# Linyou/Ced-NeRF

Measured on NVIDIA B200. Metric: train_step_rays_per_s, higher is better.
Workload: dtype f16 (MLP, tables) / f32 (marching, compositing, grads)

## Files before the change

### cednerf_b200/csrc/field_common.cuh

```cuda
#pragma once
#include "hashgrid.cuh"
#include "tc05.cuh"

struct CednerfFieldDesc {
  float aabb[6];
  float moving_step;
  int use_div_offsets;
  int time_mode;
  int time_before_sigma;
  CednerfMlpDesc f1, f2, f3;
  CednerfMlpDesc f4;
  CednerfGridLevels levels;
};

namespace {

__device__ __forceinline__ void group_sync(int group) { asm volatile("bar.sync %0, 128;" ::"r"(group + 1) : "memory"); }

__device__ __forceinline__ void run_chain(const CednerfMlpDesc& d, const uint8_t* wimg, uint8_t* abuf, uint32_t tmem_grp,
                                          uint32_t tmem_warp, uint64_t* bar, uint32_t& phase, int gtid, int group,
                                          uint8_t* save = nullptr, int64_t save_layer_stride = 0, int64_t save_row0 = 0,
                                          int save_rows = 0, uint8_t* save_in = nullptr) {

  const int L = d.n_layers;
  for (int l = 0; l < L; ++l) {
    const int K = d.dim_in[l], N = d.dim_out[l];
    if (gtid == 0) {
      tc_fence_after();
      const uint64_t ad = make_desc(smem_u32(abuf), 1, 64);
      const uint64_t bd = make_desc(smem_u32(wimg + d.image_off[l]), 1, 64);
      const uint32_t id = make_idesc(128, N, 0, 0);
      for (int k = 0; k < K / 16; ++k) umma(tmem_grp, ad + 2 * k, bd + 2 * k, id, k > 0);
      umma_commit(bar);
    }
    if (save_in && l == 0) {
      const int cpr = K >> 3;
      uint4* dst = reinterpret_cast<uint4*>(save_in + save_row0 * K * 2);
      for (int q = gtid; q < MLP_TILE * cpr; q += MLP_TILE) {
        const int r = q / cpr, c = q - r * cpr;
        if (r < save_rows) dst[q] = *reinterpret_cast<const uint4*>(abuf + swz(r, c));
      }
    }
    if (save && l > 0 && gtid == 0) {
      uint8_t* dst = save + ((int64_t)(l - 1) * save_layer_stride + (save_row0 >> 7)) * MLP_TILE_BYTES;
      asm volatile("cp.async.bulk.global.shared::cta.bulk_group [%0], [%1], %2;" ::"l"(dst), "r"(smem_u32(abuf)),
                   "r"((uint32_t)MLP_TILE_BYTES)
                   : "memory");
      asm volatile("cp.async.bulk.commit_group;" ::: "memory");
    }
    if ((gtid >> 5) == 0) {
      mbar_wait(bar, phase);
      tc_fence_after();
      tc_fence_before();
      if (save && l > 0 && gtid == 0) asm volatile("cp.async.bulk.wait_group.read 0;" ::: "memory");
    }
    group_sync(group);
    phase ^= 1;
    tc_fence_after();
    if (l < L - 1) {
#pragma unroll
      for (int cb = 0; cb < 4; ++cb) {
        uint32_t r[16];
        tmem_ld16(tmem_warp + cb * 16, r);
        tmem_ld_wait();
        uint32_t p[8];
#pragma unroll
        for (int j = 0; j < 8; ++j) p[j] = pack_relu_h2(__uint_as_float(r[2 * j]), __uint_as_float(r[2 * j + 1]));
        *reinterpret_cast<uint4*>(abuf + swz(gtid, 2 * cb)) = make_uint4(p[0], p[1], p[2], p[3]);
        *reinterpret_cast<uint4*>(abuf + swz(gtid, 2 * cb + 1)) = make_uint4(p[4], p[5], p[6], p[7]);
      }
      fence_proxy_async();
      tc_fence_before();
      group_sync(group);
    }
  }
}

__device__ __forceinline__ float rnd16(uint32_t acc_bits) { return __half2float(__float2half_rn(__uint_as_float(acc_bits))); }

template <bool EXACT = false>
__device__ __forceinline__ void time_embedding(float tv, float mvnorm, int mode, float* e ) {
  const float half_pi = 1.5707963267948966f;
  e[0] = tv;
  if (mode == 1) {
#pragma unroll
    for (int i = 0; i < 4; ++i) {
      const float tb = tv * (float)(1 << i);
      e[1 + i] = EXACT ? sinf(tb) : __sinf(tb);
      e[5 + i] = EXACT ? sinf(tb + half_pi) : __sinf(tb + half_pi);
    }
  } else {
    const float scm[4] = {0.f, 2.f, 8.f, 24.f};
#pragma unroll
    for (int i = 0; i < 4; ++i) {
      const float tb = tv * (float)(1 << i);
      const float att = EXACT ? expf(-1.f * (mvnorm * scm[i])) : __expf(-1.f * (mvnorm * scm[i]));
      e[1 + 2 * i] = (EXACT ? sinf(tb) : __sinf(tb)) * att;
      e[2 + 2 * i] = (EXACT ? sinf(tb + half_pi) : __sinf(tb + half_pi)) * att;
    }
  }
}

__device__ __noinline__ uint32_t wrapped_corner(uint32_t base, int k, uint32_t res, uint32_t r2, uint32_t size) {
  const uint32_t h = base + (uint32_t)(k & 1) + (uint32_t)((k >> 1) & 1) * res + (uint32_t)(k >> 2) * r2;
  return h >= size ? h % size : h;
}

__device__ __forceinline__ __half2 ldg_last(const __half2* p) {
  uint32_t v;
  asm("ld.global.nc.L1::evict_last.b32 %0, [%1];" : "=r"(v) : "l"(p));
  return *reinterpret_cast<__half2*>(&v);
}
__device__ __forceinline__ __half2 gather_h2(const __half2* base, uint32_t idx) {
  uint64_t addr;
  asm("mad.wide.u32 %0, %1, 4, %2;" : "=l"(addr) : "r"(idx), "l"(base));
  uint32_t v;
  asm("ld.global.nc.L1::evict_last.b32 %0, [%1];" : "=r"(v) : "l"(addr));
  return *reinterpret_cast<__half2*>(&v);
}

__device__ __forceinline__ uint64_t pack_f2(float a, float b) {
  uint64_t r;
  asm("mov.b64 %0, {%1, %2};" : "=l"(r) : "f"(a), "f"(b));
  return r;
}
__device__ __forceinline__ void unpack_f2(uint64_t v, float& a, float& b) { asm("mov.b64 {%0, %1}, %2;" : "=f"(a), "=f"(b) : "l"(v)); }
__device__ __forceinline__ uint64_t sub_f2(uint64_t a, uint64_t b) {
  uint64_t r;
  asm("sub.f32x2 %0, %1, %2;" : "=l"(r) : "l"(a), "l"(b));
  return r;
}
__device__ __forceinline__ uint64_t fma_f2(uint64_t a, uint64_t b, uint64_t c) {
  uint64_t r;
  asm("fma.rn.f32x2 %0, %1, %2, %3;" : "=l"(r) : "l"(a), "l"(b), "l"(c));
  return r;
}
__device__ __forceinline__ uint64_t h2_to_f2(__half2 h) {
  const float2 f = __half22float2(h);
  return pack_f2(f.x, f.y);
}

#ifndef HASH_PAIR_LOADS
#define HASH_PAIR_LOADS 1
#endif
#ifndef HASH_PAIR_MIN_RES
#define HASH_PAIR_MIN_RES 1024u
#endif
template <int LG>
__device__ __forceinline__ void hash_issue(const float* xn, const __half* __restrict__ table, const CednerfGridLevels& lv,
                                           int l_first, float (*frac)[3], __half2 (*v)[8]) {
#pragma unroll
  for (int a = 0; a < LG; ++a) {
// ... 154 lines not shown
```

### cednerf_b200/csrc/field_train.cu

```cuda
#include <stdlib.h>

#include "field_common.cuh"

namespace {

struct SavedLayout {
  int64_t h1, o1, in2, h2, o2, h3, h4, o4, xn, total, tiles;
};

__host__ __device__ inline SavedLayout saved_layout(const CednerfFieldDesc& d, int64_t n) {
  SavedLayout s;
  int64_t off = 0;
  const int64_t tiles = (n + MLP_TILE - 1) / MLP_TILE;
  s.tiles = tiles;
  s.h1 = off, off += (int64_t)(d.f1.n_layers - 1) * tiles * MLP_TILE_BYTES;
  s.o1 = off, off += n * 32;
  s.in2 = off, off += n * d.f2.dim_in[0] * 2;
  s.h2 = off, off += (int64_t)(d.f2.n_layers - 1) * tiles * MLP_TILE_BYTES;
  s.o2 = off, off += n * 32;
  s.h3 = off, off += (int64_t)(d.f3.n_layers - 1) * tiles * MLP_TILE_BYTES;
  s.h4 = off, off += d.f4.n_layers > 0 ? (int64_t)(d.f4.n_layers - 1) * tiles * MLP_TILE_BYTES : 0;
  s.o4 = off, off += d.f4.n_layers > 0 ? n * 64 : 0;
  s.xn = off, off += (n * 12 + 15) / 16 * 16;
  s.total = off;
  return s;
}

struct BwdWorkLayout {
  int64_t d_o2, d_in2, d_in4, g_xn, dy_lm, total;
};

__host__ __device__ inline BwdWorkLayout bwd_layout(const CednerfFieldDesc& d, int64_t n) {
  BwdWorkLayout w;
  int64_t off = 0;
  w.d_o2 = off, off += n * 32;
  w.d_in2 = off, off += n * d.f2.dim_in[0] * 2;
  w.d_in4 = off, off += n * 64;
  w.g_xn = off, off += (n * 12 + 15) / 16 * 16;
  w.dy_lm = off, off += (int64_t)d.levels.n_levels * n * 4;
  w.total = off;
  return w;
}

struct TrainArgs {
  const int64_t* ridx;
  const float* t0;
  const float* t1;
  const float* rays_o;
  const float* rays_d;
  const float* t;
  int t_stride;
  int64_t n;
  const int64_t* n_dev;
  const uint8_t* img[4];
  const __half* table;
  float* sigma;
  float* rgb;
  float* latent;
  uint8_t* selector;
  float* move;
  uint8_t* saved;
  const float* d_sigma;
  const float* d_rgb;
  const float* d_latent;
  uint8_t* work;
  float* d_params[4];
  uint32_t tmem_cols;
  int flush_tiles;
  const int32_t* order;
  CednerfFieldDesc d;
};

__device__ __forceinline__ int64_t ext_index(const TrainArgs& a, int64_t s) { return a.order ? (int64_t)a.order[s] : s; }

__device__ __forceinline__ int64_t live_count(const TrainArgs& a) {
  if (!a.n_dev) return a.n;
  const int64_t v = *a.n_dev;
  return v < a.n ? v : a.n;
}

__device__ __forceinline__ float huber(float x) {
  const float ax = fabsf(x);
  return ax < 1.f ? 0.5f * x * x : ax - 0.5f;
}

__device__ __forceinline__ void load_off(const TrainArgs& a, const SavedLayout& sl, int64_t s, float* off6) {
  const uint4 w = *reinterpret_cast<const uint4*>(a.saved + sl.o1 + s * 32);
  const uint32_t ww[4] = {w.x, w.y, w.z, w.w};
#pragma unroll
  for (int j = 0; j < 3; ++j) {
    const float2 f = __half22float2(*reinterpret_cast<const __half2*>(&ww[j]));
    off6[2 * j] = f.x;
    off6[2 * j + 1] = f.y;
  }
}

#ifdef FIELD_PHASE_CLOCKS
__device__ unsigned long long g_train_phase_clocks[12];
#define TPHASE_MARK(i)                                                           \
  do {                                                                           \
    if (gtid == 0) {                                                             \
      const long long now_ = clock64();                                          \
      atomicAdd(&g_train_phase_clocks[i], (unsigned long long)(now_ - phase_t)); \
      phase_t = now_;                                                            \
    }                                                                            \
  } while (0)
#else
#define TPHASE_MARK(i) do {} while (0)
#endif

#ifndef TRAIN_FWD_GROUPS
#define TRAIN_FWD_GROUPS 5
#endif
#ifndef TRAIN_FWD_LG
#define TRAIN_FWD_LG 4
#endif
__global__ void __launch_bounds__(TRAIN_FWD_GROUPS * 128, 1) field_train_fwd_kernel(TrainArgs a) {
  extern __shared__ __align__(1024) uint8_t smem_raw[];
  uint8_t* smem = reinterpret_cast<uint8_t*>((reinterpret_cast<uintptr_t>(smem_raw) + 1023) & ~(uintptr_t)1023);
  const CednerfFieldDesc& d = a.d;
  const bool has4 = d.f4.n_layers > 0;
  const int n_groups = blockDim.x / MLP_TILE;
  const int tid = threadIdx.x, warp = tid >> 5, group = tid / MLP_TILE, gtid = tid % MLP_TILE;
  uint8_t* w1 = smem;
  uint8_t* w2 = w1 + d.f1.image_bytes;
  uint8_t* w3 = w2 + d.f2.image_bytes;
  uint8_t* w4 = w3 + d.f3.image_bytes;
  uint8_t* abuf = reinterpret_cast<uint8_t*>(
                      (reinterpret_cast<uintptr_t>(w4 + (has4 ? d.f4.image_bytes : 0)) + 1023) & ~(uintptr_t)1023) +
                  (size_t)group * MLP_TILE_BYTES;
  __shared__ uint64_t bars[8];
  __shared__ uint32_t tmem_base_s;
  uint64_t* bar = &bars[group];
  {
    const uint8_t* src[4] = {a.img[0], a.img[1], a.img[2], a.img[3]};
    uint8_t* dst[4] = {w1, w2, w3, w4};
    const int bytes[4] = {d.f1.image_bytes, d.f2.image_bytes, d.f3.image_bytes, has4 ? d.f4.image_bytes : 0};
    for (int k = 0; k < 4; ++k)
      for (int q = tid; q < bytes[k] / 16; q += blockDim.x)
        reinterpret_cast<uint4*>(dst[k])[q] = __ldg(reinterpret_cast<const uint4*>(src[k]) + q);
  }
  const uint32_t tmem_cols = n_groups <= 1 ? 64 : (n_groups == 2 ? 128 : (n_groups <= 4 ? 256 : 512));
  if (warp == 0) tmem_alloc(&tmem_base_s, tmem_cols);
  if (gtid == 0) mbar_init(bar, 1);
  if (tid == 0) fence_barrier_init();
  fence_proxy_async();
  tc_fence_before();
  __syncthreads();
  tc_fence_after();
  const uint32_t tmem_base = tmem_base_s + 64u * (uint32_t)group;
  const uint32_t tmem_warp = tmem_base + ((uint32_t)((warp & 3) * 32) << 16);
  uint32_t phase = 0;
  const int64_t n = a.n, nl = live_count(a);
  const int64_t n_tiles = (nl + MLP_TILE - 1) / MLP_TILE;
  const int L = d.levels.n_levels;
  const uint32_t one2 = 0x3C003C00u;
  const SavedLayout sl = saved_layout(d, n);
  const int k2 = d.f2.dim_in[0];

  for (int64_t tile = blockIdx.x + (int64_t)gridDim.x * group; tile < n_tiles; tile += (int64_t)gridDim.x * n_groups) {
    const int64_t s = tile * MLP_TILE + gtid;
    const bool ok = s < nl;
    const int rows_valid = (int)((nl - tile * MLP_TILE) < MLP_TILE ? (nl - tile * MLP_TILE) : MLP_TILE);
    float x[3] = {0.f, 0.f, 0.f}, tv = 0.f;
    int64_t ray = 0;
#ifdef FIELD_PHASE_CLOCKS
    long long phase_t = clock64();
    if (gtid == 0) atomicAdd(&g_train_phase_clocks[11], 1ull);
#endif
    const int64_t e = ok ? ext_index(a, s) : 0;
    if (ok) packed_sample(a.ridx, a.t0, a.t1, a.rays_o, a.rays_d, a.t, a.t_stride, e, x, tv, ray);
    frequency_row<true>(abuf, gtid, x[0], x[1], x[2], tv);
    fence_proxy_async();
    tc_fence_before();
    group_sync(group);
    TPHASE_MARK(0);
    run_chain(d.f1, w1, abuf, tmem_base, tmem_warp, bar, phase, gtid, group, a.saved + sl.h1,
              sl.tiles, tile * MLP_TILE, rows_valid);
    TPHASE_MARK(1);
    float xn[3], mv[3], mvnorm;
    bool selector;
    {
      uint32_t r[16];
      tmem_ld16(tmem_warp, r);
      tmem_ld_wait();
      uint32_t p[8];
#pragma unroll
      for (int j = 0; j < 8; ++j) p[j] = pack_h2(__uint_as_float(r[2 * j]), __uint_as_float(r[2 * j + 1]));
      if (ok) {
        uint4* dst = reinterpret_cast<uint4*>(a.saved + sl.o1 + s * 32);
        dst[0] = make_uint4(p[0], p[1], p[2], p[3]);
        dst[1] = make_uint4(p[4], p[5], p[6], p[7]);
      }
      float off6[6];
#pragma unroll
      for (int k = 0; k < 6; ++k) off6[k] = rnd16(r[k]);
      apply_move(d, x, off6, mv, xn, selector);
      mvnorm = sqrtf(mv[0] * mv[0] + mv[1] * mv[1] + mv[2] * mv[2]);
    }
    if (ok) {
      float* xs = reinterpret_cast<float*>(a.saved + sl.xn) + 3 * s;
      xs[0] = xn[0], xs[1] = xn[1], xs[2] = xn[2];
      a.move[3 * e] = mv[0], a.move[3 * e + 1] = mv[1], a.move[3 * e + 2] = mv[2];
      a.selector[e] = (uint8_t)selector;
    }
    TPHASE_MARK(2);
    float temb[9];
    {
      auto put_word = [&](int w, uint32_t v) {
        *reinterpret_cast<uint32_t*>(abuf + swz(gtid, w >> 2) + ((w & 3) << 2)) = v;
      };
      if ((L % TRAIN_FWD_LG) == 0 && (L & 3) == 0) {
#pragma unroll 1
        for (int l0 = 0; l0 < L; l0 += TRAIN_FWD_LG) {
          uint32_t fw[TRAIN_FWD_LG];
          hash_levels<TRAIN_FWD_LG>(xn, a.table, d.levels, 0, fw, l0);
          if constexpr (TRAIN_FWD_LG >= 4) {
#pragma unroll
            for (int q = 0; q < TRAIN_FWD_LG / 4; ++q)
              *reinterpret_cast<uint4*>(abuf + swz(gtid, (l0 >> 2) + q)) = make_uint4(fw[4 * q], fw[4 * q + 1], fw[4 * q + 2], fw[4 * q + 3]);
          } else {
            *reinterpret_cast<uint2*>(abuf + swz(gtid, l0 >> 2) + ((l0 & 2) << 2)) = make_uint2(fw[0], fw[1]);
          }
        }
      } else {
#pragma unroll 1
        for (int l0 = 0; l0 < L; ++l0) {
          uint32_t f1w[1];
          hash_levels<1>(xn, a.table, d.levels, 0, f1w, l0);
          put_word(l0, f1w[0]);
        }
      }
      TPHASE_MARK(3);
      if (d.time_mode) time_embedding<true>(tv, mvnorm, d.time_mode, temb);
      int w = L;
      if (d.time_mode && d.time_before_sigma) {
#pragma unroll
        for (int j = 0; j < 4; ++j) put_word(L + j, pack_h2(temb[2 * j], temb[2 * j + 1]));
        put_word(L + 4, pack_h2(temb[8], 1.f));
        w = L + 5;
      }
      for (; 2 * w < k2; ++w) put_word(w, one2);
    }
    fence_proxy_async();
    tc_fence_before();
    group_sync(group);
    TPHASE_MARK(4);
    run_chain(d.f2, w2, abuf, tmem_base, tmem_warp, bar, phase, gtid, group, a.saved + sl.h2,
              sl.tiles, tile * MLP_TILE, rows_valid, a.saved + sl.in2);
    TPHASE_MARK(5);
    {
      uint32_t o2[16];
      tmem_ld16(tmem_warp, o2);
      tmem_ld_wait();
      uint32_t p[8];
#pragma unroll
      for (int j = 0; j < 8; ++j) p[j] = pack_h2(__uint_as_float(o2[2 * j]), __uint_as_float(o2[2 * j + 1]));
      if (ok) {
        uint4* dst = reinterpret_cast<uint4*>(a.saved + sl.o2 + s * 32);
        dst[0] = make_uint4(p[0], p[1], p[2], p[3]);
        dst[1] = make_uint4(p[4], p[5], p[6], p[7]);
        a.sigma[e] = selector ? expf(rnd16(o2[0]) - 1.f) : 0.f;
      }
      float dir[3] = {0.f, 0.f, 1.f}, feat15[15];
      if (ok) dir[0] = a.rays_d[3 * ray], dir[1] = a.rays_d[3 * ray + 1], dir[2] = a.rays_d[3 * ray + 2];
#pragma unroll
      for (int j = 0; j < 15; ++j) feat15[j] = rnd16(o2[1 + j]);
      colour_input_row(d, abuf, gtid, dir, feat15, temb);
    }
    fence_proxy_async();
    tc_fence_before();
    group_sync(group);
    TPHASE_MARK(6);
    run_chain(d.f3, w3, abuf, tmem_base, tmem_warp, bar, phase, gtid, group, a.saved + sl.h3,
              sl.tiles, tile * MLP_TILE, rows_valid);
    TPHASE_MARK(7);
    {
      uint32_t r[16];
      tmem_ld16(tmem_warp, r);
      tmem_ld_wait();
      if (ok) {
#pragma unroll
        for (int k = 0; k < 3; ++k) a.rgb[3 * e + k] = 1.f / (1.f + expf(-rnd16(r[k])));
      }
    }
    if (has4) {
      frequency_row<true>(abuf, gtid, xn[0], xn[1], xn[2], tv);
      fence_proxy_async();
      tc_fence_before();
      group_sync(group);
      TPHASE_MARK(8);
      run_chain(d.f4, w4, abuf, tmem_base, tmem_warp, bar, phase, gtid, group, a.saved + sl.h4,
                sl.tiles, tile * MLP_TILE, rows_valid);
      TPHASE_MARK(9);
#pragma unroll
      for (int cb = 0; cb < 2; ++cb) {
        uint32_t r[16];
        tmem_ld16(tmem_warp + cb * 16, r);
        tmem_ld_wait();
        if (ok) {
          uint32_t p[8];
#pragma unroll
          for (int j = 0; j < 8; ++j) p[j] = pack_h2(__uint_as_float(r[2 * j]), __uint_as_float(r[2 * j + 1]));
          uint4* dst = reinterpret_cast<uint4*>(a.saved + sl.o4 + s * 64) + 2 * cb;
          dst[0] = make_uint4(p[0], p[1], p[2], p[3]);
          dst[1] = make_uint4(p[4], p[5], p[6], p[7]);
          if (a.latent) {
            const uint4* fsrc = reinterpret_cast<const uint4*>(a.saved + sl.in2 + s * k2 * 2) + 2 * cb;
            const uint4 f0 = fsrc[0], f1 = fsrc[1];
            const uint32_t fw[8] = {f0.x, f0.y, f0.z, f0.w, f1.x, f1.y, f1.z, f1.w};
            float4* lo = reinterpret_cast<float4*>(a.latent + e * 32 + cb * 16);
            float lv[16];
#pragma unroll
            for (int j = 0; j < 8; ++j) {
              const float2 f = __half22float2(*reinterpret_cast<const __half2*>(&fw[j]));
              lv[2 * j] = selector ? huber(rnd16(r[2 * j]) - f.x) : 0.f;
              lv[2 * j + 1] = selector ? huber(rnd16(r[2 * j + 1]) - f.y) : 0.f;
            }
#pragma unroll
            for (int j = 0; j < 4; ++j) lo[j] = make_float4(lv[4 * j], lv[4 * j + 1], lv[4 * j + 2], lv[4 * j + 3]);
          }
        }
      }
    }
    tc_fence_before();
    group_sync(group);
    TPHASE_MARK(10);
  }
  tc_fence_before();
  __syncthreads();
  if (warp == 0) tmem_dealloc(tmem_base_s, tmem_cols);
}

template <int NET>
__device__ __forceinline__ const CednerfMlpDesc& net_desc(const CednerfFieldDesc& d) {
  if constexpr (NET == 1) return d.f1;
  else if constexpr (NET == 2) return d.f2;
  else if constexpr (NET == 3) return d.f3;
  else return d.f4;
}

__device__ __forceinline__ void predictor_dout(const TrainArgs& a, const SavedLayout& sl, int64_t s, int cb, uint32_t* dw) {
  const int k2 = a.d.f2.dim_in[0];
  const uint4* ps = reinterpret_cast<const uint4*>(a.saved + sl.o4 + s * 64) + 2 * cb;
  const uint4* fs = reinterpret_cast<const uint4*>(a.saved + sl.in2 + s * k2 * 2) + 2 * cb;
  const int64_t e = ext_index(a, s);
  const bool sel = a.selector[e] != 0;
#pragma unroll
  for (int c = 0; c < 2; ++c) {
    const uint4 p = ps[c], f = fs[c];
    const uint32_t pw[4] = {p.x, p.y, p.z, p.w}, fw[4] = {f.x, f.y, f.z, f.w};
    const float4 l0 = *reinterpret_cast<const float4*>(a.d_latent + e * 32 + (2 * cb + c) * 8);
    const float4 l1 = *reinterpret_cast<const float4*>(a.d_latent + e * 32 + (2 * cb + c) * 8 + 4);
    const float lg[8] = {l0.x, l0.y, l0.z, l0.w, l1.x, l1.y, l1.z, l1.w};
#pragma unroll
    for (int j = 0; j < 4; ++j) {
      const float2 pv = __half22float2(*reinterpret_cast<const __half2*>(&pw[j]));
      const float2 fv = __half22float2(*reinterpret_cast<const __half2*>(&fw[j]));
      const float d0 = sel ? lg[2 * j] * fminf(fmaxf(pv.x - fv.x, -1.f), 1.f) : 0.f;
      const float d1 = sel ? lg[2 * j + 1] * fminf(fmaxf(pv.y - fv.y, -1.f), 1.f) : 0.f;
      dw[4 * c + j] = pack_h2(d0, d1);
    }
  }
}

template <int NET>
__device__ __forceinline__ void make_dout(const TrainArgs& a, const SavedLayout& sl, const BwdWorkLayout& wl, uint8_t* tile,
                                          int row, int64_t s, bool ok) {
  const CednerfFieldDesc& d = a.d;
  uint32_t w[16];
#pragma unroll
  for (int j = 0; j < 16; ++j) w[j] = 0u;
  const int n_chunks = NET == 4 ? 4 : 2;
  if (ok) {
    if constexpr (NET == 3) {
      float g[3];
// ... 28 lines not shown
          const uint4 q = src[dim];
          const uint32_t qw[4] = {q.x, q.y, q.z, q.w};
          float acc = 0.f;
#pragma unroll
          for (int k = 0; k < 4; ++k) {
            const float2 gv = __half22float2(*reinterpret_cast<const __half2*>(&qw[k]));
            const float sc = (float)(1 << k);
            float sn, cs;
            sincospi_fast(xs[dim] * sc, sn, cs);
            acc += (gv.x * cs - gv.y * sn) * sc * 3.14159265358979323846f;
          }
          g[dim] += acc;
        }
      }
      float off6[6];
      load_off(a, sl, s, off6);
      float o[6] = {0.f, 0.f, 0.f, 0.f, 0.f, 0.f};
#pragma unroll
      for (int k = 0; k < 3; ++k) {
        const float gm = g[k] / (d.aabb[3 + k] - d.aabb[k]);
        o[k] = gm * d.moving_step;
        if (d.use_div_offsets) {
          const float th = tanhf(off6[3 + k]);
          o[3 + k] = gm * d.moving_step * (1.f - th * th);
        }
      }
      w[0] = pack_h2(o[0], o[1]);
      w[1] = pack_h2(o[2], o[3]);
      w[2] = pack_h2(o[4], o[5]);
    }
  }
#pragma unroll
  for (int c = 0; c < 4; ++c)
    if (c < n_chunks) *reinterpret_cast<uint4*>(tile + swz(row, c)) = make_uint4(w[4 * c], w[4 * c + 1], w[4 * c + 2], w[4 * c + 3]);
}

template <int NET>
__device__ __forceinline__ void make_input(const TrainArgs& a, const SavedLayout& sl, uint8_t* tile, int row, int64_t s,
                                           bool ok) {
  const CednerfFieldDesc& d = a.d;
  if (!ok) {
    const int chunks = net_desc<NET>(d).dim_in[0] / 8;
    for (int c = 0; c < chunks; ++c) *reinterpret_cast<uint4*>(tile + swz(row, c)) = make_uint4(0u, 0u, 0u, 0u);
    return;
  }
  if constexpr (NET == 2) {
    const int k2 = d.f2.dim_in[0];
    const uint4* src = reinterpret_cast<const uint4*>(a.saved + sl.in2 + s * k2 * 2);
    for (int c = 0; c < k2 / 8; ++c) *reinterpret_cast<uint4*>(tile + swz(row, c)) = src[c];
    return;
  }
  float x[3], tv;
  int64_t ray;
  packed_sample(a.ridx, a.t0, a.t1, a.rays_o, a.rays_d, a.t, a.t_stride, ext_index(a, s), x, tv, ray);
  if constexpr (NET == 1) {
    frequency_row<true>(tile, row, x[0], x[1], x[2], tv);
  } else if constexpr (NET == 4) {
    const float* xs = reinterpret_cast<const float*>(a.saved + sl.xn) + 3 * s;
    frequency_row<true>(tile, row, xs[0], xs[1], xs[2], tv);
  } else {
    float temb[9];
    if (d.time_mode && !d.time_before_sigma) {
      float off6[6], mv[3], xn[3];
      bool sel;
      load_off(a, sl, s, off6);
      apply_move(d, x, off6, mv, xn, sel);
      time_embedding<true>(tv, sqrtf(mv[0] * mv[0] + mv[1] * mv[1] + mv[2] * mv[2]), d.time_mode, temb);
    }
    const uint4* src = reinterpret_cast<const uint4*>(a.saved + sl.o2 + s * 32);
    const uint4 q0 = src[0], q1 = src[1];
    const uint32_t qw[8] = {q0.x, q0.y, q0.z, q0.w, q1.x, q1.y, q1.z, q1.w};
    float o2[16];
#pragma unroll
    for (int j = 0; j < 8; ++j) {
      const float2 f = __half22float2(*reinterpret_cast<const __half2*>(&qw[j]));
      o2[2 * j] = f.x, o2[2 * j + 1] = f.y;
    }
    const float dir[3] = {a.rays_d[3 * ray], a.rays_d[3 * ray + 1], a.rays_d[3 * ray + 2]};
    colour_input_row(d, tile, row, dir, o2 + 1, temb);
  }
}

#define BWD_GROUPS 4
#define BWD_GROUP_SMEM (3 * MLP_TILE_BYTES)

template <int NET>
__global__ void __launch_bounds__(BWD_GROUPS * MLP_TILE, 1) field_bwd_kernel(TrainArgs a) {
  extern __shared__ __align__(1024) uint8_t smem_raw[];
  uint8_t* smem = reinterpret_cast<uint8_t*>((reinterpret_cast<uintptr_t>(smem_raw) + 1023) & ~(uintptr_t)1023);
  const CednerfMlpDesc& d = net_desc<NET>(a.d);
  const int n_groups = blockDim.x / MLP_TILE;
  const int tid = threadIdx.x, warp = tid >> 5, lane = tid & 31, group = tid / MLP_TILE, gtid = tid % MLP_TILE;
  uint8_t* wsm = smem;
  uint8_t* gsm = smem + ((d.image_bytes + 1023) & ~1023) + (size_t)group * BWD_GROUP_SMEM;
  uint8_t* gbuf = gsm;
  uint8_t* ibuf[2] = {gsm + MLP_TILE_BYTES, gsm + 2 * MLP_TILE_BYTES};
  __shared__ uint64_t bars[BWD_GROUPS];
  __shared__ uint32_t tmem_base_s;
  uint64_t* bar = &bars[group];
  const int64_t n = a.n, nl = live_count(a);
  const SavedLayout sl = saved_layout(a.d, n);
  const BwdWorkLayout wl = bwd_layout(a.d, n);
  const uint8_t* image = a.img[NET - 1];
  const uint8_t* hidden = a.saved + (NET == 1 ? sl.h1 : (NET == 2 ? sl.h2 : (NET == 3 ? sl.h3 : sl.h4)));
  __shared__ uint64_t lbars[BWD_GROUPS];
  uint64_t* lbar = &lbars[group];
  uint32_t lphase = 0;
  auto fetch_tile = [&](uint8_t* dst, int layer, int64_t tile_idx) {
    if (gtid == 0) {
      asm volatile("mbarrier.arrive.expect_tx.shared::cta.b64 _, [%0], %1;" ::"r"(smem_u32(lbar)), "r"((uint32_t)MLP_TILE_BYTES)
                   : "memory");
      asm volatile("cp.async.bulk.shared::cluster.global.mbarrier::complete_tx::bytes [%0], [%1], %2, [%3];" ::"r"(smem_u32(dst)),
                   "l"(hidden + ((int64_t)layer * sl.tiles + tile_idx) * MLP_TILE_BYTES), "r"((uint32_t)MLP_TILE_BYTES),
                   "r"(smem_u32(lbar))
                   : "memory");
    }
  };
  auto await_tile = [&]() {
    mbar_wait(lbar, lphase);
    lphase ^= 1;
  };
  float* d_params = a.d_params[NET - 1];
  const int L = d.n_layers;
  for (int q = tid; q < d.image_bytes / 16; q += blockDim.x)
    reinterpret_cast<uint4*>(wsm)[q] = __ldg(reinterpret_cast<const uint4*>(image) + q);
  if (warp == 0) tmem_alloc(&tmem_base_s, a.tmem_cols);
  if (gtid == 0) {
    mbar_init(bar, 1);
    mbar_init(lbar, 1);
  }
  if (tid == 0) fence_barrier_init();
  fence_proxy_async();
  tc_fence_before();
  __syncthreads();
  if (gtid == 0) fence_barrier_init();
  tc_fence_after();
  const uint32_t tmem_base = tmem_base_s;
  const uint32_t tmem_grp = tmem_base + 64u * (uint32_t)group;
  const uint32_t tmem_warp = tmem_grp + ((uint32_t)((warp & 3) * 32) << 16);
  const uint32_t wg_base = tmem_base + 64u * (uint32_t)n_groups;
  const uint32_t wg_warp = wg_base + ((uint32_t)((warp & 3) * 32) << 16);
  if (group == 0) {
    for (int cb = 0; cb < 4 * ((L + 1) / 2); ++cb) tmem_st16_fill(wg_warp + cb * 16, 0u);
    tmem_st_wait();
  }
  tc_fence_before();
  __syncthreads();
  tc_fence_after();
  uint32_t phase = 0;
  const int64_t n_tiles = (nl + MLP_TILE - 1) / MLP_TILE;
  const bool want_dx = NET != 1;

  auto flush_wgrad = [&](bool rezero) {
    if (group == 0) {
      for (int l = 0; l < L; ++l) {
        const int K_in = d.dim_in[l], N_out = d.dim_out[l];
        const int half = l & 1;
        const int m = warp * 16 + (lane & 15);
        for (int cb = 0; cb < K_in / 16; ++cb) {
          uint32_t r[16];
          tmem_ld16(wg_warp + 64u * (uint32_t)(l >> 1) + cb * 16, r);
          tmem_ld_wait();
          if ((lane >> 4) == half && m < N_out) {
            float* dst = d_params + d.param_off[l] + m * K_in + cb * 16;
#pragma unroll
            for (int j = 0; j < 16; ++j) atomicAdd(dst + j, __uint_as_float(r[j]));
          }
        }
      }
      if (rezero) {
        for (int cb = 0; cb < 4 * ((L + 1) / 2); ++cb) tmem_st16_fill(wg_warp + cb * 16, 0u);
        tmem_st_wait();
      }
      tc_fence_before();
    }
  };
  const int64_t stride = (int64_t)gridDim.x * n_groups;
  const int64_t first = blockIdx.x + (int64_t)gridDim.x * group;
  const int64_t n_iter = (n_tiles - blockIdx.x + stride - 1) / stride;
  for (int64_t it = 0; it < n_iter; ++it) {
    const int64_t tile = first + it * stride;
    if (a.flush_tiles > 0 && it > 0 && (it % a.flush_tiles) == 0) {
      tc_fence_before();
      __syncthreads();
      tc_fence_after();
      flush_wgrad(true);
      __syncthreads();
      tc_fence_after();
    }
    if (tile >= n_tiles) continue;
    const int64_t row0 = tile * MLP_TILE;
    const int rows_valid = (int)((nl - row0) < MLP_TILE ? (nl - row0) : MLP_TILE);
    const int64_t s = row0 + gtid;
    const bool ok = gtid < rows_valid;
    if (L > 1) fetch_tile(ibuf[0], L - 2, tile);
    else make_input<NET>(a, sl, ibuf[0], gtid, s, ok);
    make_dout<NET>(a, sl, wl, gbuf, gtid, s, ok);
    if (L > 1) await_tile();
    fence_proxy_async();
    tc_fence_before();
    group_sync(group);
    int cur = 0;
    for (int l = L - 1; l >= 0; --l) {
      const int K_in = d.dim_in[l], N_out = d.dim_out[l];
      const bool need_dgrad = (l > 0) || want_dx;
      if (gtid == 0) {
        tc_fence_after();
        {
          const uint64_t ad = make_desc(smem_u32(gbuf), 64, 64);
          const uint64_t bd = make_desc(smem_u32(ibuf[cur]), 64, 64);
          const uint32_t id = make_idesc(64, K_in, 1, 1);
          const uint32_t acc = wg_base + 64u * (uint32_t)(l >> 1) + ((uint32_t)((l & 1) * 16) << 16);
          for (int k = 0; k < MLP_TILE / 16; ++k) umma(acc, ad + 128 * k, bd + 128 * k, id, 1u);
        }
        if (need_dgrad) {
          const uint64_t ad = make_desc(smem_u32(gbuf), 1, 64);
          const uint64_t bd = make_desc(smem_u32(wsm + d.image_off[l]), 64, 64);
          const uint32_t id = make_idesc(128, K_in, 0, 1);
          for (int k = 0; k < N_out / 16; ++k) umma(tmem_grp, ad + 2 * k, bd + 128 * k, id, k > 0);
        }
        umma_commit(bar);
      }
      if (l > 0) {
        if (l > 1) fetch_tile(ibuf[cur ^ 1], l - 2, tile);
        else make_input<NET>(a, sl, ibuf[cur ^ 1], gtid, s, ok);
      }
      if ((gtid >> 5) == 0) {
        mbar_wait(bar, phase);
        tc_fence_after();
        tc_fence_before();
      }
      group_sync(group);
      phase ^= 1;
      tc_fence_after();
      if (l > 0) {
        const uint8_t* act = ibuf[cur];
#pragma unroll
        for (int cb = 0; cb < 4; ++cb) {
          uint32_t r[16];
          tmem_ld16(tmem_warp + cb * 16, r);
          tmem_ld_wait();
          const uint4 m0 = *reinterpret_cast<const uint4*>(act + swz(gtid, 2 * cb));
          const uint4 m1 = *reinterpret_cast<const uint4*>(act + swz(gtid, 2 * cb + 1));
          const uint32_t mw[8] = {m0.x, m0.y, m0.z, m0.w, m1.x, m1.y, m1.z, m1.w};
          uint32_t p[8];
#pragma unroll
          for (int j = 0; j < 8; ++j) {
            const unsigned keep = __hgt2_mask(*reinterpret_cast<const __half2*>(&mw[j]), __float2half2_rn(0.f));
            p[j] = pack_h2(__uint_as_float(r[2 * j]), __uint_as_float(r[2 * j + 1])) & keep;
          }
          *reinterpret_cast<uint4*>(gbuf + swz(gtid, 2 * cb)) = make_uint4(p[0], p[1], p[2], p[3]);
          *reinterpret_cast<uint4*>(gbuf + swz(gtid, 2 * cb + 1)) = make_uint4(p[4], p[5], p[6], p[7]);
        }
      } else if (want_dx) {
        if constexpr (NET == 3) {
          uint32_t r0[16], r1[16];
          tmem_ld16(tmem_warp, r0);
          tmem_ld16(tmem_warp + 16, r1);
          tmem_ld_wait();
          if (ok) {
            float v[16];
            v[0] = 0.f;
#pragma unroll
            for (int j = 1; j <= 12; ++j) v[j] = __uint_as_float(r0[3 + j]);
#pragma unroll
            for (int j = 13; j <= 15; ++j) v[j] = __uint_as_float(r1[j - 13]);
            uint4* dst = reinterpret_cast<uint4*>(a.work + wl.d_o2 + s * 32);
            dst[0] = make_uint4(pack_h2(v[0], v[1]), pack_h2(v[2], v[3]), pack_h2(v[4], v[5]), pack_h2(v[6], v[7]));
            dst[1] = make_uint4(pack_h2(v[8], v[9]), pack_h2(v[10], v[11]), pack_h2(v[12], v[13]), pack_h2(v[14], v[15]));
          }
        } else {
          uint8_t* out = a.work + (NET == 2 ? wl.d_in2 + s * K_in * 2 : wl.d_in4 + s * 64);
          for (int cb = 0; cb < K_in / 16; ++cb) {
            uint32_t r[16];
            tmem_ld16(tmem_warp + cb * 16, r);
            tmem_ld_wait();
            if (ok) {
              uint32_t p[8];
#pragma unroll
              for (int j = 0; j < 8; ++j) p[j] = pack_h2(__uint_as_float(r[2 * j]), __uint_as_float(r[2 * j + 1]));
              if constexpr (NET == 2) {
                if (a.d.f4.n_layers > 0 && a.d_latent && cb < 2) {
                  uint32_t dw[8];
                  predictor_dout(a, sl, s, cb, dw);
#pragma unroll
                  for (int j = 0; j < 8; ++j) {
                    const __half2 q = __hsub2(*reinterpret_cast<const __half2*>(&p[j]), *reinterpret_cast<const __half2*>(&dw[j]));
                    p[j] = *reinterpret_cast<const uint32_t*>(&q);
                  }
                }
                uint32_t* lm = reinterpret_cast<uint32_t*>(a.work + wl.dy_lm);
#pragma unroll
                for (int j = 0; j < 8; ++j)
                  if (8 * cb + j < a.d.levels.n_levels) lm[(int64_t)(8 * cb + j) * n + s] = p[j];
              } else {
                reinterpret_cast<uint4*>(out)[2 * cb] = make_uint4(p[0], p[1], p[2], p[3]);
                reinterpret_cast<uint4*>(out)[2 * cb + 1] = make_uint4(p[4], p[5], p[6], p[7]);
              }
            }
          }
        }
      }
      if (l > 1) await_tile();
      fence_proxy_async();
      tc_fence_before();
      group_sync(group);
      cur ^= 1;
    }
  }
  tc_fence_before();
  __syncthreads();
  tc_fence_after();
  flush_wgrad(false);
  __syncthreads();
  if (warp == 0) tmem_dealloc(tmem_base, a.tmem_cols);
}

__global__ void __launch_bounds__(256) hashgrid_bwd_input_lm_kernel(const float* __restrict__ xn, int64_t n,
                                                                    const __half* __restrict__ table, CednerfGridLevels lv,
                                                                    const __half2* __restrict__ dy_lm, float* __restrict__ g_x,
                                                                    const int64_t* __restrict__ n_dev) {
  const int64_t s = (int64_t)blockIdx.x * blockDim.x + threadIdx.x;
  if (s >= n || (n_dev && s >= *n_dev)) return;
  const float x[3] = {xn[3 * s], xn[3 * s + 1], xn[3 * s + 2]};
  float gx[3] = {0.f, 0.f, 0.f};
  const int L = lv.n_levels;
  auto level_terms = [&](const float* f, const __half2* v, int l) {
    const float2 d = __half22float2(dy_lm[(int64_t)l * n + s]);
    float dot[8];
#pragma unroll
    for (int k = 0; k < 8; ++k) {
      const float2 t = __half22float2(v[k]);
      dot[k] = t.x * d.x + t.y * d.y;
    }
    const float wx[2] = {1.f - f[0], f[0]}, wy[2] = {1.f - f[1], f[1]}, wz[2] = {1.f - f[2], f[2]};
    float a[3] = {0.f, 0.f, 0.f};
#pragma unroll
    for (int q = 0; q < 2; ++q)
#pragma unroll
      for (int p = 0; p < 2; ++p) {
        a[0] += wy[p] * wz[q] * (dot[1 + 2 * p + 4 * q] - dot[0 + 2 * p + 4 * q]);
        a[1] += wx[p] * wz[q] * (dot[p + 2 + 4 * q] - dot[p + 0 + 4 * q]);
        a[2] += wx[p] * wy[q] * (dot[p + 2 * q + 4] - dot[p + 2 * q]);
      }
    const float sc = lv.scale[l];
    gx[0] += a[0] * sc, gx[1] += a[1] * sc, gx[2] += a[2] * sc;
  };
  int l0 = 0;
#pragma unroll 1
  for (; l0 + 2 <= L; l0 += 2) {
    float frac[2][3];
    __half2 v[2][8];
    hash_issue<2>(x, table, lv, l0, frac, v);
    level_terms(frac[0], v[0], l0);
    level_terms(frac[1], v[1], l0 + 1);
  }
  if (l0 < L) {
    float frac[1][3];
    __half2 v[1][8];
    hash_issue<1>(x, table, lv, l0, frac, v);
    level_terms(frac[0], v[0], l0);
  }
  g_x[3 * s] = gx[0], g_x[3 * s + 1] = gx[1], g_x[3 * s + 2] = gx[2];
}

constexpr int BWD_SMEM_MAX = 226 * 1024;

int check_train_desc(const CednerfFieldDesc* d) {
  if (!d) return 0;
  const int L = d->levels.n_levels;
  if (L < 1 || L > 16 || d->time_mode < 0 || d->time_mode > 2) return 0;
  const CednerfMlpDesc* nets[4] = {&d->f1, &d->f2, &d->f3, &d->f4};
  for (int k = 0; k < 4; ++k) {
    const int nl = nets[k]->n_layers;
    if (k == 3 && nl == 0) continue;
    if (nl < 1 || nl > MLP_MAX_LAYERS) return 0;
  }
  if (d->f1.dim_in[0] != 32 || d->f1.dim_out[d->f1.n_layers - 1] != 16) return 0;
  const int in2 = 2 * L + ((d->time_mode && d->time_before_sigma) ? 9 : 0);
  if (d->f2.dim_in[0] != (in2 + 15) / 16 * 16 || d->f2.dim_out[d->f2.n_layers - 1] != 16) return 0;
  const int in3 = 19 + ((d->time_mode && !d->time_before_sigma) ? 9 : 0);
  if (d->f3.dim_in[0] != (in3 + 15) / 16 * 16 || d->f3.dim_out[d->f3.n_layers - 1] != 16) return 0;
  if (d->f4.n_layers > 0 && (L != 16 || d->f4.dim_in[0] != 32 || d->f4.dim_out[d->f4.n_layers - 1] != 32)) return 0;
  return 1;
}

template <int NET>
int launch_bwd(TrainArgs a, cudaStream_t st) {
  static CednerfOncePerDevice configured;
  if (int e = cednerf_opt_in_smem(field_bwd_kernel<NET>, BWD_SMEM_MAX, configured, "cednerf_field_train_bwd")) return e;
  const CednerfMlpDesc& d = NET == 1 ? a.d.f1 : (NET == 2 ? a.d.f2 : (NET == 3 ? a.d.f3 : a.d.f4));
  int groups = BWD_GROUPS;
  if (const char* env = getenv("CEDNERF_BWD_GROUPS")) {
    const int g = atoi(env);
    if (g >= 1 && g < groups) groups = g;
  }
  const int fixed = ((d.image_bytes + 1023) & ~1023) + 2048;
  while (groups > 1 && (fixed + groups * BWD_GROUP_SMEM > BWD_SMEM_MAX || 64 * (groups + (d.n_layers + 1) / 2) > 512)) --groups;
  uint32_t cols = 64u * (uint32_t)(groups + (d.n_layers + 1) / 2), alloc = 64;
  while (alloc < cols) alloc <<= 1;
  a.tmem_cols = alloc;
  a.flush_tiles = 0;
  if (const char* env = getenv("CEDNERF_BWD_FLUSH_TILES")) a.flush_tiles = atoi(env);
  const int64_t tiles = (a.n + MLP_TILE - 1) / MLP_TILE;
  const int64_t max_ctas = (int64_t)cednerf_num_sms();
  field_bwd_kernel<NET><<<(unsigned)(tiles < max_ctas ? tiles : max_ctas), groups * MLP_TILE, fixed + groups * BWD_GROUP_SMEM, st>>>(a);
  return 0;
}

}

extern "C" int cednerf_hashgrid_bwd_table_lm_dev(const float* x, int x_stride, int64_t n, const int64_t* n_device,
                                                 const CednerfGridLevels* levels, const void* dy_lm_f16, float* g_table,
                                                 void* stream);
extern "C" int cednerf_hashgrid_bwd(const float* x, int x_stride, int64_t n, const void* table_f16,
                                    const CednerfGridLevels* levels, const void* dy, int dy_stride, int dy_is_f16,
                                    float* g_table, float* g_x, void* stream);

CEDNERF_EXPORT int64_t cednerf_field_saved_bytes(const CednerfFieldDesc* desc, int64_t n) {
  return desc ? saved_layout(*desc, n).total : -1;
}
CEDNERF_EXPORT int64_t cednerf_field_bwd_workspace_bytes(const CednerfFieldDesc* desc, int64_t n) {
  return desc ? bwd_layout(*desc, n).total : -1;
}

CEDNERF_EXPORT int cednerf_field_train_fwd(const int64_t* ray_indices, const float* t_starts, const float* t_ends,
                                           const float* rays_o, const float* rays_d, const float* timestamps,
                                           int t_stride, int64_t n, const void* image_deform, const void* image_density,
                                           const void* image_colour, const void* image_predict, const void* table_f16,
                                           const CednerfFieldDesc* desc, float* sigma, float* rgb, float* latent,
                                           uint8_t* selector, float* move, void* saved, const int32_t* sample_order,
                                           const int64_t* n_device, void* stream) {
  CEDNERF_REQUIRE(check_train_desc(desc), "bad field descriptor");
  CEDNERF_REQUIRE(n >= 0 && ray_indices && t_starts && t_ends && rays_o && rays_d && timestamps && sigma && rgb &&
                      selector && move && saved,
                  "bad arguments");
  CEDNERF_REQUIRE(desc->f4.n_layers == 0 || image_predict, "feature predictor image missing");
  if (n == 0) return 0;
  const int n_groups = TRAIN_FWD_GROUPS;
  const int smem = desc->f1.image_bytes + desc->f2.image_bytes + desc->f3.image_bytes +
                   (desc->f4.n_layers > 0 ? desc->f4.image_bytes : 0) + n_groups * MLP_TILE_BYTES + 2048;
  CEDNERF_REQUIRE(smem <= 224 * 1024, "networks too large for the fused kernel");
  static CednerfOncePerDevice configured;
  if (int e = cednerf_opt_in_smem(field_train_fwd_kernel, 224 * 1024, configured, "cednerf_field_train_fwd")) return e;
  TrainArgs a{};
  a.ridx = ray_indices, a.t0 = t_starts, a.t1 = t_ends, a.rays_o = rays_o, a.rays_d = rays_d, a.t = timestamps;
  a.t_stride = t_stride, a.n = n, a.n_dev = n_device;
  a.img[0] = (const uint8_t*)image_deform, a.img[1] = (const uint8_t*)image_density;
  a.img[2] = (const uint8_t*)image_colour, a.img[3] = (const uint8_t*)image_predict;
  a.table = (const __half*)table_f16;
  a.sigma = sigma, a.rgb = rgb, a.latent = desc->f4.n_layers > 0 ? latent : nullptr, a.selector = selector, a.move = move;
  a.saved = (uint8_t*)saved, a.order = sample_order;
  a.d = *desc;
  const int64_t tiles = (n + MLP_TILE - 1) / MLP_TILE;
  const int64_t ctas = tiles;
  const int64_t max_ctas = (int64_t)cednerf_num_sms();
  field_train_fwd_kernel<<<(unsigned)(ctas < max_ctas ? ctas : max_ctas), n_groups * MLP_TILE, smem, (cudaStream_t)stream>>>(a);
  return cednerf_check_launch("cednerf_field_train_fwd");
}

CEDNERF_EXPORT int cednerf_field_train_bwd(const int64_t* ray_indices, const float* t_starts, const float* t_ends,
                                           const float* rays_o, const float* rays_d, const float* timestamps,
                                           int t_stride, int64_t n, const void* image_deform, const void* image_density,
                                           const void* image_colour, const void* image_predict, const void* table_f16,
                                           const CednerfFieldDesc* desc, const float* sigma, const float* rgb,
                                           const uint8_t* selector, const void* saved, const float* d_sigma,
                                           const float* d_rgb, const float* d_latent, void* work, float* d_params_deform,
                                           float* d_params_density, float* d_params_colour, float* d_params_predict,
                                           float* g_table, int phase, const int32_t* sample_order,
                                           const int64_t* n_device, void* stream) {
  CEDNERF_REQUIRE(check_train_desc(desc), "bad field descriptor");
  CEDNERF_REQUIRE(phase >= 0 && phase <= 2, "phase: 0 all, 1 up to the table gradient, 2 the rest");
  CEDNERF_REQUIRE(n >= 0 && ray_indices && t_starts && t_ends && rays_o && rays_d && timestamps && rgb && selector &&
                      saved && d_sigma && d_rgb && work && d_params_deform && d_params_density && d_params_colour &&
                      g_table,
                  "bad arguments");
  const bool has4 = desc->f4.n_layers > 0 && d_latent != nullptr;
  CEDNERF_REQUIRE(!has4 || (image_predict && d_params_predict), "feature predictor buffers missing");
  if (n == 0) return 0;
  cudaStream_t st = (cudaStream_t)stream;
  TrainArgs a{};
  a.ridx = ray_indices, a.t0 = t_starts, a.t1 = t_ends, a.rays_o = rays_o, a.rays_d = rays_d, a.t = timestamps;
  a.t_stride = t_stride, a.n = n, a.n_dev = n_device;
  a.img[0] = (const uint8_t*)image_deform, a.img[1] = (const uint8_t*)image_density;
  a.img[2] = (const uint8_t*)image_colour, a.img[3] = (const uint8_t*)image_predict;
  a.table = (const __half*)table_f16;
  a.sigma = const_cast<float*>(sigma), a.rgb = const_cast<float*>(rgb), a.selector = const_cast<uint8_t*>(selector);
  a.saved = (uint8_t*)saved, a.order = sample_order;
  a.d_sigma = d_sigma, a.d_rgb = d_rgb, a.d_latent = d_latent, a.work = (uint8_t*)work;
// ... 35 lines not shown
```

Before: 54.23 million.

## Recompute MLP hidden activations in backward instead of saving them

The forward pass no longer stores each MLP's hidden-layer tiles to global memory with bulk async copies. The backward kernel re-runs the forward chain on-chip into per-group shared-memory slots, using ping-pong recomputation for 4-layer nets, and overlaps the dout construction through a hook. This removes the global write and read traffic for hidden activations and shrinks the saved buffer, at the cost of extra tensor-core GEMMs and a different shared-memory footprint per group in backward.

```diff
diff --git a/cednerf_b200/csrc/field_common.cuh b/cednerf_b200/csrc/field_common.cuh
--- a/cednerf_b200/csrc/field_common.cuh
+++ b/cednerf_b200/csrc/field_common.cuh
@@ -17,17 +17,24 @@
 
 __device__ __forceinline__ void group_sync(int group) { asm volatile("bar.sync %0, 128;" ::"r"(group + 1) : "memory"); }
 
+struct NoHook {
+  __device__ void operator()() const {}
+};
+template <class Hook = NoHook>
 __device__ __forceinline__ void run_chain(const CednerfMlpDesc& d, const uint8_t* wimg, uint8_t* abuf, uint32_t tmem_grp,
                                           uint32_t tmem_warp, uint64_t* bar, uint32_t& phase, int gtid, int group,
-                                          uint8_t* save = nullptr, int64_t save_layer_stride = 0, int64_t save_row0 = 0,
-                                          int save_rows = 0, uint8_t* save_in = nullptr) {
-
-  const int L = d.n_layers;
+                                          int64_t save_row0 = 0, int save_rows = 0, uint8_t* save_in = nullptr,
+                                          uint8_t* keep = nullptr, int keep_slots = 0, int n_run = -1,
+                                          int hook_layer = -1, Hook hook = Hook()) {
+  const int L = n_run >= 0 ? n_run : (keep ? d.n_layers - 1 : d.n_layers);
+  auto kept = [&](int l) { return keep + (size_t)(keep_slots ? l % keep_slots : l) * MLP_TILE_BYTES; };
   for (int l = 0; l < L; ++l) {
     const int K = d.dim_in[l], N = d.dim_out[l];
+    const uint8_t* src = (keep && l > 0) ? kept(l - 1) : abuf;
+    uint8_t* out = keep ? kept(l) : abuf;
     if (gtid == 0) {
       tc_fence_after();
-      const uint64_t ad = make_desc(smem_u32(abuf), 1, 64);
+      const uint64_t ad = make_desc(smem_u32(src), 1, 64);
       const uint64_t bd = make_desc(smem_u32(wimg + d.image_off[l]), 1, 64);
       const uint32_t id = make_idesc(128, N, 0, 0);
       for (int k = 0; k < K / 16; ++k) umma(tmem_grp, ad + 2 * k, bd + 2 * k, id, k > 0);
@@ -41,23 +48,16 @@
         if (r < save_rows) dst[q] = *reinterpret_cast<const uint4*>(abuf + swz(r, c));
       }
     }
-    if (save && l > 0 && gtid == 0) {
-      uint8_t* dst = save + ((int64_t)(l - 1) * save_layer_stride + (save_row0 >> 7)) * MLP_TILE_BYTES;
-      asm volatile("cp.async.bulk.global.shared::cta.bulk_group [%0], [%1], %2;" ::"l"(dst), "r"(smem_u32(abuf)),
-                   "r"((uint32_t)MLP_TILE_BYTES)
-                   : "memory");
-      asm volatile("cp.async.bulk.commit_group;" ::: "memory");
-    }
+    if (l == hook_layer) hook();
     if ((gtid >> 5) == 0) {
       mbar_wait(bar, phase);
       tc_fence_after();
       tc_fence_before();
-      if (save && l > 0 && gtid == 0) asm volatile("cp.async.bulk.wait_group.read 0;" ::: "memory");
     }
     group_sync(group);
     phase ^= 1;
     tc_fence_after();
-    if (l < L - 1) {
+    if (keep || l < L - 1) {
 #pragma unroll
       for (int cb = 0; cb < 4; ++cb) {
         uint32_t r[16];
@@ -66,8 +66,8 @@
         uint32_t p[8];
 #pragma unroll
         for (int j = 0; j < 8; ++j) p[j] = pack_relu_h2(__uint_as_float(r[2 * j]), __uint_as_float(r[2 * j + 1]));
-        *reinterpret_cast<uint4*>(abuf + swz(gtid, 2 * cb)) = make_uint4(p[0], p[1], p[2], p[3]);
-        *reinterpret_cast<uint4*>(abuf + swz(gtid, 2 * cb + 1)) = make_uint4(p[4], p[5], p[6], p[7]);
+        *reinterpret_cast<uint4*>(out + swz(gtid, 2 * cb)) = make_uint4(p[0], p[1], p[2], p[3]);
+        *reinterpret_cast<uint4*>(out + swz(gtid, 2 * cb + 1)) = make_uint4(p[4], p[5], p[6], p[7]);
       }
       fence_proxy_async();
       tc_fence_before();
diff --git a/cednerf_b200/csrc/field_train.cu b/cednerf_b200/csrc/field_train.cu
--- a/cednerf_b200/csrc/field_train.cu
+++ b/cednerf_b200/csrc/field_train.cu
@@ -5,21 +5,15 @@
 namespace {
 
 struct SavedLayout {
-  int64_t h1, o1, in2, h2, o2, h3, h4, o4, xn, total, tiles;
+  int64_t o1, in2, o2, o4, xn, total;
 };
 
 __host__ __device__ inline SavedLayout saved_layout(const CednerfFieldDesc& d, int64_t n) {
   SavedLayout s;
   int64_t off = 0;
-  const int64_t tiles = (n + MLP_TILE - 1) / MLP_TILE;
-  s.tiles = tiles;
-  s.h1 = off, off += (int64_t)(d.f1.n_layers - 1) * tiles * MLP_TILE_BYTES;
   s.o1 = off, off += n * 32;
   s.in2 = off, off += n * d.f2.dim_in[0] * 2;
-  s.h2 = off, off += (int64_t)(d.f2.n_layers - 1) * tiles * MLP_TILE_BYTES;
   s.o2 = off, off += n * 32;
-  s.h3 = off, off += (int64_t)(d.f3.n_layers - 1) * tiles * MLP_TILE_BYTES;
-  s.h4 = off, off += d.f4.n_layers > 0 ? (int64_t)(d.f4.n_layers - 1) * tiles * MLP_TILE_BYTES : 0;
   s.o4 = off, off += d.f4.n_layers > 0 ? n * 64 : 0;
   s.xn = off, off += (n * 12 + 15) / 16 * 16;
   s.total = off;
@@ -175,8 +169,7 @@
     tc_fence_before();
     group_sync(group);
     TPHASE_MARK(0);
-    run_chain(d.f1, w1, abuf, tmem_base, tmem_warp, bar, phase, gtid, group, a.saved + sl.h1,
-              sl.tiles, tile * MLP_TILE, rows_valid);
+    run_chain(d.f1, w1, abuf, tmem_base, tmem_warp, bar, phase, gtid, group);
     TPHASE_MARK(1);
     float xn[3], mv[3], mvnorm;
     bool selector;
@@ -246,8 +239,8 @@
     tc_fence_before();
     group_sync(group);
     TPHASE_MARK(4);
-    run_chain(d.f2, w2, abuf, tmem_base, tmem_warp, bar, phase, gtid, group, a.saved + sl.h2,
-              sl.tiles, tile * MLP_TILE, rows_valid, a.saved + sl.in2);
+    run_chain(d.f2, w2, abuf, tmem_base, tmem_warp, bar, phase, gtid, group, tile * MLP_TILE, rows_valid,
+              a.saved + sl.in2);
     TPHASE_MARK(5);
     {
       uint32_t o2[16];
@@ -272,8 +265,7 @@
     tc_fence_before();
     group_sync(group);
     TPHASE_MARK(6);
-    run_chain(d.f3, w3, abuf, tmem_base, tmem_warp, bar, phase, gtid, group, a.saved + sl.h3,
-              sl.tiles, tile * MLP_TILE, rows_valid);
+    run_chain(d.f3, w3, abuf, tmem_base, tmem_warp, bar, phase, gtid, group);
     TPHASE_MARK(7);
     {
       uint32_t r[16];
@@ -290,8 +282,7 @@
       tc_fence_before();
       group_sync(group);
       TPHASE_MARK(8);
-      run_chain(d.f4, w4, abuf, tmem_base, tmem_warp, bar, phase, gtid, group, a.saved + sl.h4,
-                sl.tiles, tile * MLP_TILE, rows_valid);
+      run_chain(d.f4, w4, abuf, tmem_base, tmem_warp, bar, phase, gtid, group);
       TPHASE_MARK(9);
 #pragma unroll
       for (int cb = 0; cb < 2; ++cb) {
@@ -486,7 +477,7 @@
 }
 
 #define BWD_GROUPS 4
-#define BWD_GROUP_SMEM (3 * MLP_TILE_BYTES)
+__host__ __device__ constexpr int bwd_group_tiles(int n_layers) { return n_layers < 3 ? n_layers + 1 : (n_layers == 4 ? 3 : n_layers); }
 
 template <int NET>
 __global__ void __launch_bounds__(BWD_GROUPS * MLP_TILE, 1) field_bwd_kernel(TrainArgs a) {
@@ -495,10 +486,15 @@
   const CednerfMlpDesc& d = net_desc<NET>(a.d);
   const int n_groups = blockDim.x / MLP_TILE;
   const int tid = threadIdx.x, warp = tid >> 5, lane = tid & 31, group = tid / MLP_TILE, gtid = tid % MLP_TILE;
+  const int L = d.n_layers;
   uint8_t* wsm = smem;
-  uint8_t* gsm = smem + ((d.image_bytes + 1023) & ~1023) + (size_t)group * BWD_GROUP_SMEM;
+  uint8_t* gsm = smem + ((d.image_bytes + 1023) & ~1023) + (size_t)group * bwd_group_tiles(L) * MLP_TILE_BYTES;
   uint8_t* gbuf = gsm;
-  uint8_t* ibuf[2] = {gsm + MLP_TILE_BYTES, gsm + 2 * MLP_TILE_BYTES};
+  const bool pingpong = L == 4;
+  uint8_t* hid = gsm + MLP_TILE_BYTES;
+  uint8_t* ibuf = pingpong ? hid : gsm + (size_t)(L < 3 ? L : L - 1) * MLP_TILE_BYTES;
+  const bool in_own_slot = L < 3;
+  const int in_step = pingpong ? 2 : 1;
   __shared__ uint64_t bars[BWD_GROUPS];
   __shared__ uint32_t tmem_base_s;
   uint64_t* bar = &bars[group];
@@ -506,38 +502,15 @@
   const SavedLayout sl = saved_layout(a.d, n);
   const BwdWorkLayout wl = bwd_layout(a.d, n);
   const uint8_t* image = a.img[NET - 1];
-  const uint8_t* hidden = a.saved + (NET == 1 ? sl.h1 : (NET == 2 ? sl.h2 : (NET == 3 ? sl.h3 : sl.h4)));
-  __shared__ uint64_t lbars[BWD_GROUPS];
-  uint64_t* lbar = &lbars[group];
-  uint32_t lphase = 0;
-  auto fetch_tile = [&](uint8_t* dst, int layer, int64_t tile_idx) {
-    if (gtid == 0) {
-      asm volatile("mbarrier.arrive.expect_tx.shared::cta.b64 _, [%0], %1;" ::"r"(smem_u32(lbar)), "r"((uint32_t)MLP_TILE_BYTES)
-                   : "memory");
-      asm volatile("cp.async.bulk.shared::cluster.global.mbarrier::complete_tx::bytes [%0], [%1], %2, [%3];" ::"r"(smem_u32(dst)),
-                   "l"(hidden + ((int64_t)layer * sl.tiles + tile_idx) * MLP_TILE_BYTES), "r"((uint32_t)MLP_TILE_BYTES),
-                   "r"(smem_u32(lbar))
-                   : "memory");
-    }
-  };
-  auto await_tile = [&]() {
-    mbar_wait(lbar, lphase);
-    lphase ^= 1;
-  };
   float* d_params = a.d_params[NET - 1];
-  const int L = d.n_layers;
   for (int q = tid; q < d.image_bytes / 16; q += blockDim.x)
     reinterpret_cast<uint4*>(wsm)[q] = __ldg(reinterpret_cast<const uint4*>(image) + q);
   if (warp == 0) tmem_alloc(&tmem_base_s, a.tmem_cols);
-  if (gtid == 0) {
-    mbar_init(bar, 1);
-    mbar_init(lbar, 1);
-  }
+  if (gtid == 0) mbar_init(bar, 1);
   if (tid == 0) fence_barrier_init();
   fence_proxy_async();
   tc_fence_before();
   __syncthreads();
-  if (gtid == 0) fence_barrier_init();
   tc_fence_after();
   const uint32_t tmem_base = tmem_base_s;
   const uint32_t tmem_grp = tmem_base + 64u * (uint32_t)group;
@@ -597,22 +570,31 @@
     const int rows_valid = (int)((nl - row0) < MLP_TILE ? (nl - row0) : MLP_TILE);
     const int64_t s = row0 + gtid;
     const bool ok = gtid < rows_valid;
-    if (L > 1) fetch_tile(ibuf[0], L - 2, tile);
-    else make_input<NET>(a, sl, ibuf[0], gtid, s, ok);
-    make_dout<NET>(a, sl, wl, gbuf, gtid, s, ok);
-    if (L > 1) await_tile();
+    if (L > 1) {
+      uint8_t* src = in_own_slot ? ibuf : gbuf;
+      make_input<NET>(a, sl, src, gtid, s, ok);
+      fence_proxy_async();
+      tc_fence_before();
+      group_sync(group);
+      run_chain(d, wsm, src, tmem_grp, tmem_warp, bar, phase, gtid, group, 0, 0, nullptr, hid, pingpong ? 2 : 0, -1,
+                in_own_slot ? 0 : 1, [&]() { make_dout<NET>(a, sl, wl, gbuf, gtid, s, ok); });
+    } else {
+      make_input<NET>(a, sl, ibuf, gtid, s, ok);
+      make_dout<NET>(a, sl, wl, gbuf, gtid, s, ok);
+    }
     fence_proxy_async();
     tc_fence_before();
     group_sync(group);
-    int cur = 0;
     for (int l = L - 1; l >= 0; --l) {
       const int K_in = d.dim_in[l], N_out = d.dim_out[l];
       const bool need_dgrad = (l > 0) || want_dx;
+      const uint8_t* act = l == 0 ? ibuf
+                           : hid + (size_t)(pingpong ? (l == 1 ? 1 : (l - 1) & 1) : l - 1) * MLP_TILE_BYTES;
       if (gtid == 0) {
         tc_fence_after();
         {
           const uint64_t ad = make_desc(smem_u32(gbuf), 64, 64);
-          const uint64_t bd = make_desc(smem_u32(ibuf[cur]), 64, 64);
+          const uint64_t bd = make_desc(smem_u32(act), 64, 64);
           const uint32_t id = make_idesc(64, K_in, 1, 1);
           const uint32_t acc = wg_base + 64u * (uint32_t)(l >> 1) + ((uint32_t)((l & 1) * 16) << 16);
           for (int k = 0; k < MLP_TILE / 16; ++k) umma(acc, ad + 128 * k, bd + 128 * k, id, 1u);
@@ -625,10 +607,7 @@
         }
         umma_commit(bar);
       }
-      if (l > 0) {
-        if (l > 1) fetch_tile(ibuf[cur ^ 1], l - 2, tile);
-        else make_input<NET>(a, sl, ibuf[cur ^ 1], gtid, s, ok);
-      }
+      if (l == in_step && !in_own_slot) make_input<NET>(a, sl, ibuf, gtid, s, ok);
       if ((gtid >> 5) == 0) {
         mbar_wait(bar, phase);
         tc_fence_after();
@@ -638,7 +617,6 @@
       phase ^= 1;
       tc_fence_after();
       if (l > 0) {
-        const uint8_t* act = ibuf[cur];
 #pragma unroll
         for (int cb = 0; cb < 4; ++cb) {
           uint32_t r[16];
@@ -705,11 +683,11 @@
           }
         }
       }
-      if (l > 1) await_tile();
       fence_proxy_async();
       tc_fence_before();
       group_sync(group);
-      cur ^= 1;
+      if (pingpong && l == 2)
+        run_chain(d, wsm, ibuf, tmem_grp, tmem_warp, bar, phase, gtid, group, 0, 0, nullptr, hid + MLP_TILE_BYTES, 1, 1);
     }
   }
   tc_fence_before();
@@ -800,7 +778,8 @@
     if (g >= 1 && g < groups) groups = g;
   }
   const int fixed = ((d.image_bytes + 1023) & ~1023) + 2048;
-  while (groups > 1 && (fixed + groups * BWD_GROUP_SMEM > BWD_SMEM_MAX || 64 * (groups + (d.n_layers + 1) / 2) > 512)) --groups;
+  const int group_smem = bwd_group_tiles(d.n_layers) * MLP_TILE_BYTES;
+  while (groups > 1 && (fixed + groups * group_smem > BWD_SMEM_MAX || 64 * (groups + (d.n_layers + 1) / 2) > 512)) --groups;
   uint32_t cols = 64u * (uint32_t)(groups + (d.n_layers + 1) / 2), alloc = 64;
   while (alloc < cols) alloc <<= 1;
   a.tmem_cols = alloc;
@@ -808,7 +787,7 @@
   if (const char* env = getenv("CEDNERF_BWD_FLUSH_TILES")) a.flush_tiles = atoi(env);
   const int64_t tiles = (a.n + MLP_TILE - 1) / MLP_TILE;
   const int64_t max_ctas = (int64_t)cednerf_num_sms();
-  field_bwd_kernel<NET><<<(unsigned)(tiles < max_ctas ? tiles : max_ctas), groups * MLP_TILE, fixed + groups * BWD_GROUP_SMEM, st>>>(a);
+  field_bwd_kernel<NET><<<(unsigned)(tiles < max_ctas ? tiles : max_ctas), groups * MLP_TILE, fixed + groups * group_smem, st>>>(a);
   return 0;
 }
 
```

New measurement: 54.39 million, median of 6. No clear change (+0.3%).
